# ALRhub/fancy_gym

Measured on AMD Instinct MI355X. Metric: MP trajectories/sec (7-DoF, 5 basis, 100 steps) at 1/2/4/8 GPUs; % roofline, higher is better.
Workload: dtype f32; 1 GPU; cfg2: ProDMP 7-DoF, 5 basis(+goal), 100 steps, exp phase tau=1.5, alpha=10; trajectory (pos, vel) + PD tracking-controller actions, fused; batch_per_gpu=4096, global_batch=4096, launch=hipgraph

## Files before the change

fancy_gym_amd/_lib.py:

```python
from __future__ import annotations

import ctypes as C
import os
from typing import Optional

_HERE = os.path.dirname(os.path.abspath(__file__))
LIB_PATH = os.environ.get("MPK_LIB") or os.path.join(_HERE, "libmpk.so")

MPK_ABI_VERSION = 4
MP_TYPES = {"promp": 0, "dmp": 1, "prodmp": 2}
PHASE_TYPES = {"linear": 0, "exp": 1}
BASIS_TYPES = {"rbf": 0, "zero_rbf": 1, "prodmp": 2}
CTRL_TYPES = {"motor": 0, "velocity": 1, "position": 2}
PLANT_TYPES = {"static": 0, "double_integrator": 1, "velocity_direct": 2}

MPK_EINVAL, MPK_ENOTIMPL, MPK_EHIP, MPK_ERANGE, MPK_ENODEV, MPK_ECOMM = -1, -2, -3, -4, -5, -6
MPK_COMM_ID_BYTES = 128
MPK_LOGPROB_MAX_OBS = 64
MPK_OPT_AUTO = -1
RELATIVE_GOAL_MODES = {"before_scale": 0, "after_scale": 1}
GOAL_OFFSET_MODES = {"ignore": 0, "add": 1}
SINGLE_RBF_MODES = {"unit_gap": 0, "refuse": 1}
DMP_FIRST_SAMPLE_MODES = {"init": 0, "step": 1}
REWARD_TYPES = {None: 0, "none": 0, "simple_reacher": 1}
AGG_MODES = {"sum": 0, "mean": 1, "last": 2}
OPTION_KEYS = ("mapping", "bulk", "quad", "pd_quad", "write_through", "ipw", "phase", "phase_table", "phase_chunk",
               "pd_simple", "split", "lds_pad", "pipe", "flat", "phase_flat", "ring", "ring_np", "ring_ns", "ring_m", "ring_dbg", "ring_parts", "tiles_wpb", "serial_order", "ring_nc", "pd_generic", "dmp_response", "ablations", "ring_tb", "pd_helper", "phase_waves", "phase_split", "phase_pipe", "pd_pipe", "hole_sampled", "vjp_generic")


class MPKLibraryError(RuntimeError):
    """libmpk.so is missing / failed to load / reported a HIP failure."""


class mpk_config(C.Structure):
    _fields_ = [
        ("abi_version", C.c_int32), ("device", C.c_int32),
        ("mp_type", C.c_int32), ("phase_type", C.c_int32), ("basis_type", C.c_int32),
        ("num_dof", C.c_int32), ("num_basis", C.c_int32), ("num_basis_outside", C.c_int32),
        ("num_basis_zero_start", C.c_int32), ("num_basis_zero_goal", C.c_int32),
        ("learn_tau", C.c_int32), ("learn_delay", C.c_int32),
        ("auto_scale_basis", C.c_int32), ("relative_goal", C.c_int32),
        ("disable_goal", C.c_int32), ("disable_weights", C.c_int32),
        ("pre_compute_length_factor", C.c_int32),
        ("relative_goal_mode", C.c_int32), ("goal_offset_mode", C.c_int32), ("single_rbf_mode", C.c_int32),
        ("dmp_first_sample", C.c_int32), ("reserved0", C.c_int32),
        ("tau", C.c_double), ("delay", C.c_double), ("alpha_phase", C.c_double),
        ("tau_bound", C.c_double * 2), ("delay_bound", C.c_double * 2),
        ("basis_bandwidth_factor", C.c_double), ("basis_alpha", C.c_double), ("basis_dt", C.c_double),
        ("weights_scale", C.c_double), ("goal_scale", C.c_double), ("dmp_alpha", C.c_double),
        ("dt", C.c_double), ("duration", C.c_double), ("goal_offset", C.c_double),
# ... 116 lines not shown
    "mpk_reacher_reset": (C.c_int, [_vp, C.POINTER(mpk_reacher_reset_task), _vp, _vp, _vp, _vp, _vp, _vp, _vp, _vp, _vp, _vp,
                                    _i32, _vp]),
    "mpk_reacher_observation": (C.c_int, [_vp, C.POINTER(mpk_obs_cfg), _vp, _vp, _vp, _vp, _vp, _i32, _vp]),
    "mpk_reacher_step_observations": (C.c_int, [_vp, C.POINTER(mpk_obs_cfg), C.POINTER(mpk_rollout_cfg), _vp, _vp, _vp, _vp, _vp, _vp,
                                                _vp, _vp, _vp, _vp, _i32, _i32, _vp]),
    "mpk_replan_advance": (C.c_int, [_vp, _vp, _vp, _vp, _vp, _i32, _i32, _i32, _i32, _i32, _vp]),
    "mpk_traj_validity": (C.c_int, [_vp, _vp, _vp, _vp, _vp, _i32, _vp, _vp, _vp, _i32, _i32, _vp]),
    "mpk_traj_validity_penalty": (C.c_int, [_vp, _vp, _vp, _vp, _vp, _i32, _vp, _vp, _vp, _vp, _i32, _i32, _vp]),
    "mpk_prodmp_tables": (C.c_int, [_vp, _vp, _vp, _vp, _vp, _vp, _vp, _vp]),
    "mpk_prodmp_indices": (C.c_int, [_vp, _dbl, _vp, _vp, _vp]),
    "mpk_scaled_basis": (C.c_int, [_vp, _vp, _i32, _vp, _vp]),
    "mpk_selftest_division": (C.c_int, [_vp, C.c_float, C.c_uint32, C.c_uint64, C.POINTER(C.c_uint64), _vp]),
    "mpk_host_prodmp_tables": (C.c_int, [C.POINTER(mpk_config), _vp, _vp, _vp, _vp, _vp, _vp, _vp, _vp]),
    "mpk_host_rbf": (C.c_int, [C.POINTER(mpk_config), _vp, _vp]),
    "mpk_host_times": (C.c_int, [_dbl, _dbl, _vp, _i32]),
    "mpk_host_num_params": (C.c_int, [C.POINTER(mpk_config)]),
    "mpk_comm_unique_id": (C.c_int, [_vp]),
    "mpk_comm_create": (C.c_int, [_vp, _i32, _i32, _i32, C.POINTER(_vp)]),
    "mpk_comm_rank": (C.c_int, [_vp]),
    "mpk_comm_world": (C.c_int, [_vp]),
    "mpk_allgather": (C.c_int, [_vp, _vp, _vp, C.c_int64, _vp]),
    "mpk_comm_destroy": (None, [_vp]),
    "mpk_last_kernel": (C.c_char_p, [_vp]),
    "mpk_reacher_autoreset": (C.c_int, [_vp, C.POINTER(mpk_reacher_reset_task), C.POINTER(mpk_obs_cfg), _vp, _vp, _vp, _vp, _vp, _vp,
                                        _vp, _vp, _vp, _vp, _vp, _vp, _vp, _vp, _i32, _vp]),
    "mpk_reacher_env_step": (C.c_int, [_vp, C.POINTER(mpk_env_step_task), C.POINTER(mpk_reacher_reset_task), _vp, _vp, _vp, _vp, _vp,
                                       _vp, _vp, _vp, _vp, _vp, _vp, _vp, _vp, _vp, _vp, _i32, _vp]),
    "mpk_trajectory_vjp": (C.c_int, [_vp, _vp, _vp, _dbl, _vp, _vp, _vp, _i32, _vp]),
    "mpk_reacher_rollout_vjp": (C.c_int, [_vp, C.POINTER(mpk_rollout_cfg), _vp, _vp, _vp, _vp, _vp, _vp, _vp, _i32, _vp, _vp, _vp,
                                          _vp, _vp, _vp, _vp, _vp, _i32, _i32, _vp]),
    "mpk_episode_return_vjp": (C.c_int, [_vp, _vp, _vp, _vp, _dbl, C.POINTER(mpk_rollout_cfg), _vp, _vp, _vp, _vp, _vp, _i32, _i32,
                                         _vp, _vp, _vp, _vp, _vp, _vp, _vp, _vp, _vp, _vp, _vp, _i32, _vp]),
    "mpk_hole_reacher_rollout_vjp": (C.c_int, [_vp, C.POINTER(mpk_rollout_cfg), _vp, _vp, _vp, _vp, _vp, _vp, C.POINTER(mpk_hole_task),
                                               _vp, _vp, _i32, _vp, _vp, _vp, _vp, _vp, _vp, _vp, _vp, _vp, _i32, _i32, _vp]),
    "mpk_reacher_rollout_vjp_cond": (C.c_int, [_vp, C.POINTER(mpk_rollout_cfg), _vp, _vp, _vp, _vp, _vp, _vp, _vp, _i32, _vp, _vp, _vp,
                                               _vp, _vp, _vp, _vp, _vp, _vp, _vp, _i32, _i32, _vp]),
    "mpk_episode_return_vjp_cond": (C.c_int, [_vp, _vp, _vp, _vp, _dbl, C.POINTER(mpk_rollout_cfg), _vp, _vp, _vp, _vp, _vp, _i32, _i32,
                                              _vp, _vp, _vp, _vp, _vp, _vp, _vp, _vp, _vp, _vp, _vp, _vp, _vp, _i32, _vp]),
    "mpk_hole_reacher_rollout_vjp_cond": (C.c_int, [_vp, C.POINTER(mpk_rollout_cfg), _vp, _vp, _vp, _vp, _vp, _vp,
                                                    C.POINTER(mpk_hole_task), _vp, _vp, _i32, _vp, _vp, _vp, _vp, _vp, _vp, _vp, _vp, _vp,
                                                    _vp, _vp, _i32, _i32, _vp]),
    "mpk_trajectory_fit": (C.c_int, [_vp, _vp, _vp, _vp, _vp, _dbl, _dbl, _vp, _i32, _vp]),
    "mpk_trajectory_phase_fit": (C.c_int, [_vp, _vp, _vp, _vp, _vp, _vp, _dbl, _dbl, _vp, _i32, _vp]),
    "mpk_fit_status": (C.c_int, [_vp, C.POINTER(C.c_int32), _vp]),
    "mpk_trajectory_std": (C.c_int, [_vp, _vp, _dbl, _vp, _vp, _i32, _vp]),
    "mpk_trajectory_condition": (C.c_int, [_vp, _vp, _vp, _vp, _vp, _dbl, C.POINTER(C.c_int32), _i32, _vp, _vp, _vp, _vp, _vp, _vp,
# ... 117 lines not shown
```

fancy_gym_amd/csrc/mpk_host.cpp:

```cpp
#include <hip/hip_runtime.h>
#include <dlfcn.h>

#include <cmath>
#include <cstdio>
#include <cstring>
#include <limits>
#include <map>
#include <mutex>
#include <set>

#include "mpk_internal.h"

namespace mpk {

static thread_local std::string g_err;
void set_error(const std::string& msg) { g_err = msg; }

const char* cond_variant_name(const char* plain) {
    static std::mutex m;
    static std::set<std::string> pool;
    std::lock_guard<std::mutex> lock(m);
    return pool.insert(std::string(plain) + " + cond").first->c_str();
}

// ... 181 lines not shown
    double* d_tab = nullptr;
    std::vector<float> rows32;
    float* d_rows32 = nullptr;
    int rows32_stride = 0;
    float* d_times = nullptr;
    int32_t* d_flag = nullptr;
    unsigned* d_tickets = nullptr;
    unsigned ticket_next = 0;
    std::vector<unsigned> ticket_free;
    std::map<std::pair<unsigned long long, uintptr_t>, unsigned> ticket_of;
    std::mutex ticket_mu;
    int* h_fault = nullptr;
    int* d_fault = nullptr;
    int32_t* d_idx = nullptr;
    int idx_cap = 0;
    static constexpr int kCache = 64;
    CacheEntry cache[kCache];
    DevCfg dev_resp{};
    bool resp_ok = false;
    CacheEntry cache_resp[kCache];
    std::string kernel_name_buf;
    uint64_t stamp = 0;
    const char* last_kernel = "";
    Tuning tune;
    float* d_pre = nullptr;
    size_t pre_cap = 0;
    static constexpr int kFitCache = 16;
    FitEntry fit_cache[kFitCache];
    int32_t* d_fit_status = nullptr;
};

static Tuning effective_tuning(const Handle* h);

static int check_cfg(const mpk_config& c) {
    if (c.abi_version != MPK_ABI_VERSION) { set_error("mpk_config.abi_version mismatch"); return MPK_EINVAL; }
    if (c.mp_type < 0 || c.mp_type > 2) { set_error("unknown mp_type"); return MPK_EINVAL; }
    if (c.phase_type < 0 || c.phase_type > 1) { set_error("unknown phase_type"); return MPK_EINVAL; }
    if (c.basis_type < 0 || c.basis_type > 2) { set_error("unknown basis_type"); return MPK_EINVAL; }
    if (c.num_dof < 0) { set_error("num_dof must be >= 0"); return MPK_EINVAL; }
    if (c.num_basis < 1) { set_error("num_basis must be >= 1 (basis length 0 is not implemented upstream)"); return MPK_EINVAL; }
    if (c.basis_type == MPK_BASIS_PRODMP && c.phase_type != MPK_PHASE_EXP) {
        set_error("prodmp basis requires the exp phase generator");
        return MPK_EINVAL;
    }
    if ((c.mp_type == MPK_MP_PRODMP) != (c.basis_type == MPK_BASIS_PRODMP)) {
        set_error("prodmp trajectory generator and prodmp basis generator must be used together");
// ... 434 lines not shown
    return prealloc_cache(h);
}

namespace {
struct OptKey { const char* name; int Tuning::*field; int64_t lo, hi; };
const OptKey kOptKeys[] = {
    {"mapping", &Tuning::mapping, 0, 2},         {"bulk", &Tuning::bulk, 0, 2},
    {"quad", &Tuning::quad, 0, 4},               {"pd_quad", &Tuning::pd_quad, 0, 3},
    {"write_through", &Tuning::write_through, 0, 1}, {"ipw", &Tuning::ipw, 0, 1 << 20},
    {"phase", &Tuning::phase, 0, 1},             {"phase_table", &Tuning::phase_table, 0, 1},
    {"phase_chunk", &Tuning::phase_chunk, 0, 16}, {"pd_simple", &Tuning::pd_simple, 0, 1},
    {"split", &Tuning::split, 0, 1},             {"lds_pad", &Tuning::lds_pad, 0, 48},
    {"pipe", &Tuning::pipe, 0, 1},               {"flat", &Tuning::flat, 0, 1},
    {"phase_flat", &Tuning::phase_flat, 0, 1},   {"ring", &Tuning::ring, 0, 2},
    {"ring_np", &Tuning::ring_np, 1, 14},        {"ring_ns", &Tuning::ring_ns, 1, 8},
    {"ring_m", &Tuning::ring_m, 1, 8},           {"ring_dbg", &Tuning::ring_dbg, 0, 255},
    {"ring_parts", &Tuning::ring_parts, 1, 8},   {"tiles_wpb", &Tuning::tiles_wpb, 1, 8},
    {"serial_order", &Tuning::serial_order, 0, 2}, {"ring_nc", &Tuning::ring_nc, 1, 6},
    {"pd_generic", &Tuning::pd_generic, 0, 1},   {"dmp_response", &Tuning::dmp_response, 0, 1},
    {"ablations", &Tuning::ablations, 0, 1},     {"ring_tb", &Tuning::ring_tb, 1, 64},
    {"pd_helper", &Tuning::pd_helper, 0, 1},     {"phase_waves", &Tuning::phase_waves, 1, 32},
    {"phase_split", &Tuning::phase_split, 1, 64},   {"phase_pipe", &Tuning::phase_pipe, 0, 1},
    {"pd_pipe", &Tuning::pd_pipe, 0, 1},         {"hole_sampled", &Tuning::hole_sampled, 0, 1},
    {"vjp_generic", &Tuning::vjp_generic, 0, 1},
};
const OptKey* find_opt(const char* key) {
    if (!key) return nullptr;
    for (const OptKey& k : kOptKeys)
        if (std::strcmp(k.name, key) == 0) return &k;
    return nullptr;
}
}

namespace mpk {
static Tuning effective_tuning(const Handle* h) {
    Tuning t = g_tune;
    for (const OptKey& k : kOptKeys)
        if (h->tune.*(k.field) >= 0) t.*(k.field) = h->tune.*(k.field);
    return t;
}
}

int mpk_set_option(mpk_handle hh, const char* key, int64_t value) {
    const OptKey* k = find_opt(key);
    if (!k) { set_error(std::string("unknown option key: ") + (key ? key : "(null)")); return MPK_EINVAL; }
    if (value != MPK_OPT_AUTO && (value < k->lo || value > k->hi)) {
        set_error(std::string("option value out of range for ") + key);
// ... 114 lines not shown
    out->check_td = g->check_tau_delay ? 1 : 0;
    if (out->check_td && h->dev.P < 2) { set_error("validity gate: check_tau_delay needs at least two parameters per episode"); return MPK_EINVAL; }
    out->tau_b[0] = g->tau_bound[0]; out->tau_b[1] = g->tau_bound[1];
    out->delay_b[0] = g->delay_bound[0]; out->delay_b[1] = g->delay_bound[1];
    out->raw_params = g->raw_params; out->valid = g->valid; out->penalty = g->penalty;
    return MPK_OK;
}

static int fill_replan(const mpk_replan_state* st, const float* init_pos, const float* init_vel, ReplanDev* rp) {
    if (!st || !st->traj_steps || !st->plan_steps || !st->done || !st->seg_len) { set_error("NULL replanning state"); return MPK_EINVAL; }
    if ((st->cond_pos == nullptr) != (st->cond_vel == nullptr)) { set_error("cond_pos and cond_vel go together"); return MPK_EINVAL; }
    if (st->every < 1 || st->horizon < 1) { set_error("every and horizon must be >= 1"); return MPK_EINVAL; }
    if (st->cond_pos && (st->cond_pos == init_pos || st->cond_vel == init_vel)) { set_error("cond_pos / cond_vel must not alias init_pos / init_vel"); return MPK_EINVAL; }
    rp->traj_steps = st->traj_steps; rp->plan_steps = st->plan_steps; rp->done = st->done; rp->seg_len = st->seg_len;
    rp->done_out = st->done_out; rp->cond_pos = st->cond_pos; rp->cond_vel = st->cond_vel;
    rp->every = st->every; rp->max_planning_times = st->max_planning_times; rp->horizon = st->horizon;
    return MPK_OK;
}

static LaunchSite launch_site(Handle* h, const Tuning& tune, void* stream) {
    LaunchSite at;
    at.num_cu = h->num_cu; at.tune = tune; at.stream = stream; at.kernel_name = &h->last_kernel;
    at.fault = h->d_fault; at.range_flag = h->d_flag;
    return at;
}

static void report_kernel(Handle* h, const char* name, bool resp) {
    h->kernel_name_buf = name;
    const size_t at = resp ? h->kernel_name_buf.find("prodmp") : std::string::npos;
    if (at != std::string::npos) h->kernel_name_buf.replace(at, 6, "dmp_resp");
    h->last_kernel = h->kernel_name_buf.c_str();
}

static int phase_fused_common(Handle* h, const TrajRequest& q, void* stream) {
    if (!q.params || !q.init_pos || !q.init_vel) { set_error("NULL buffer"); return MPK_EINVAL; }
    if (const int fr = pending_ring_fault(h); fr != MPK_OK) return fr;
    return launch_phase_fused(h->dev, q, launch_site(h, effective_tuning(h), stream));
}

static int traj_common(Handle* h, const TrajRequest& req, void* stream) {
    if (req.B < 0) { set_error("B must be >= 0"); return MPK_EINVAL; }
    if (req.B == 0 || h->dev.D == 0) return MPK_OK;
    if (!req.params || !req.init_pos || !req.init_vel || !req.pos || !req.vel) { set_error("NULL buffer"); return MPK_EINVAL; }
    MPK_ON_DEVICE(h->cfg.device);
    if (const int fr = pending_ring_fault(h); fr != MPK_OK) return fr;
    TrajRequest q = req;
// ... 1399 lines not shown
    if (count < 0) { set_error("count must be >= 0"); return MPK_EINVAL; }
    if (count == 0) return MPK_OK;
    if (!send || !recv) { set_error("NULL buffer"); return MPK_EINVAL; }
    Comm* c = reinterpret_cast<Comm*>(cc);
    MPK_ON_DEVICE(c->device);
    const int rc = rccl().AllGather(send, recv, (size_t)count, kNcclFloat, c->nccl, (hipStream_t)stream);
    if (rc != 0) return rccl_fail("ncclAllGather", rc);
    return MPK_OK;
}

void mpk_comm_destroy(mpk_comm cc) {
    if (!cc) return;
    Comm* c = reinterpret_cast<Comm*>(cc);
    DeviceGuard guard(c->device);
    if (c->nccl) (void)rccl().CommDestroy(c->nccl);
    delete c;
}

const char* mpk_last_kernel(mpk_handle hh) {
    if (!hh) return "";
    return reinterpret_cast<Handle*>(hh)->last_kernel;
}

}
```

fancy_gym_amd/csrc/mpk_internal.h:

```cpp
#pragma once
#include <cstdint>
#include <string>
#include <vector>

#include "mpk.h"

namespace mpk {

constexpr int kMaxKP = 16;
constexpr int kMaxD = 16;
constexpr int kMaxDofArgs = 32;

struct HostTables {
    int n_total = 0;
    std::vector<double> centers, bw;
    int n_pc = 0;
    float scaled_dt = 0.f;
    std::vector<double> y1, y2, dy1, dy2, pos_basis, vel_basis, scale;
};

void build_rbf(const mpk_config& c, HostTables& t);
void build_prodmp(const mpk_config& c, HostTables& t);
std::vector<float> build_times(double duration, int T);
int steps_for(double duration, double dt);

struct Tuning {
    int mapping = -1, bulk = -1, quad = -1, pd_quad = -1, write_through = -1, ipw = -1, phase = -1, phase_table = -1,
        phase_chunk = -1, pd_simple = -1, split = -1, lds_pad = -1, pipe = -1, flat = -1, phase_flat = -1,
        ring = -1, ring_np = -1, ring_ns = -1, ring_m = -1, ring_dbg = -1, ring_parts = -1, tiles_wpb = -1, serial_order = -1, ring_nc = -1,
        pd_generic = -1, dmp_response = -1, ablations = -1, ring_tb = -1, pd_helper = -1, phase_waves = -1, phase_split = -1, phase_pipe = -1, pd_pipe = -1,
        hole_sampled = -1, vjp_generic = -1;
};

struct DevCfg {
    int mp_type, phase_type, basis_type;
    int D, nb, n_total, zs;
    int KT, KP;
    int P, Kloc, off;
    int T;
    int learn_tau, learn_delay, relative_goal, disable_goal, disable_weights;
    int rbf_uniform;
    int relgoal_before_scale;
    int dmp_resp;
    int goal_off_on;
    float goal_offset;
    int n_pc, len_factor;
    float tau, delay, alpha_phase, scaled_dt;
    float tau_lo, tau_hi, delay_lo, delay_hi;
    float ws, gs, dmp_alpha, dmp_beta;
    const double* tab;
    const float* rows32;
    int rows32_stride;
    const float* base_times;
    float t_last;
// ... 50 lines not shown
    const int32_t* step0 = nullptr;
    double* ret = nullptr;
    int32_t* seg_out = nullptr;
};
struct TrajRequest {
    const float *params = nullptr, *init_pos = nullptr, *init_vel = nullptr;
    const float* init_time = nullptr;
    float init_time_shared = 0.f;
    float *pos = nullptr, *vel = nullptr, *actions = nullptr;
    const RolloutDev* rc = nullptr;
    const double *c_pos = nullptr, *c_vel = nullptr;
    double *q_state = nullptr, *qd_state = nullptr;
    const int32_t* n_steps = nullptr;
    const ReplanDev* rp = nullptr;
    const GateDev* gate = nullptr;
    EpisodeAsk ep;
    int B = 0;
};
struct LaunchSite {
    int num_cu = 0;
    Tuning tune;
    void* stream = nullptr;
    const char** kernel_name = nullptr;
    unsigned* ticket = nullptr;
    int* fault = nullptr;
    int32_t* range_flag = nullptr;
};

int launch_build_shared(const DevCfg& c, float init_time, const SharedTables& st, int32_t* idx_out,
                        int32_t* range_flag, void* stream);
int launch_traj_shared(const DevCfg& c, const SharedTables& st, const TrajRequest& q, const LaunchSite& at);
int launch_episode_return(const DevCfg& c, const SharedTables& st, const TrajRequest& q, const LaunchSite& at);
int launch_reward_aggregate(const double* rewards, const int32_t* seg_len, int agg, double* out, int B, int T, void* stream);
int launch_traj_wide(const DevCfg& c, const SharedTables& st, const TrajRequest& q, const LaunchSite& at);
int launch_traj_vjp(const DevCfg& c, const SharedTables& st, const float* g_pos, const float* g_vel, float* g_params, float* g_init_pos,
                    float* g_init_vel, int B, int num_cu, void* stream, const char** kernel_name, const Tuning& tune);
int launch_traj_rows(const DevCfg& c, const TrajRequest& q, const LaunchSite& at);
int launch_pd_rollout(const RolloutDev& rc, int D, const float* des_pos, const float* des_vel, double* q,
                      double* qd, const int32_t* n_steps, float* actions, int B, int T, void* stream,
                      const Tuning& tune, int* fault = nullptr);
bool phase_fused_capable(const DevCfg& c);
int launch_phase_fused(const DevCfg& c, const TrajRequest& q, const LaunchSite& at);
int fast_rows_floats(const DevCfg& c);
int fast_rows_stride(const DevCfg& c);
int launch_fast_rows_table(const DevCfg& c, float* out, void* stream);
int launch_dmp_prestep(const DevCfg& c, const TrajRequest& q, float* pos1, float* vel1, void* stream);
// ... 215 lines not shown
```

fancy_gym_amd/csrc/mpk_tile.h:

```cpp
#pragma once
#include "mpk_dev.h"

namespace mpk {

struct TrajArgs {
    DevCfg c;
    const float* A;
    const float* aux;
    int TS;
    const float* params;
    const float* init_pos;
    const float* init_vel;
    float* pos;
    float* vel;
    float* actions;
    const double* c_pos;
    const double* c_vel;
    int B, sh, G, vec_ok;
    int pitch, cps, shifted, td3;
    unsigned inv_cps;
    unsigned nrt_magic;
    int gstride;
    int wt;
    int flat_img;
// ... 625 lines not shown
                const f32x2 v2 = {head ? d1[2] : d1[0], head ? d1[3] : d1[1]};
                if (SP) store8<WT>(a.pos + go + o, p2);
                if (SV) store8<WT>(a.vel + go + o, v2);
                if (SA) {
                    const f32x2 a2 = {head ? d2[2] : d2[0], head ? d2[3] : d2[1]};
                    store8<WT>(a.actions + go + o, a2);
                }
            } else {
#pragma unroll
                for (int e = 0; e < 4; ++e) {
                    if (c0 + e >= lo && c0 + e < hi) {
                        if (SP) store4<WT>(a.pos + go + e, d0[e]);
                        if (SV) store4<WT>(a.vel + go + e, d1[e]);
                        if (SA) store4<WT>(a.actions + go + e, d2[e]);
                    }
                }
            }
        }
    } else {
        store_tile_generic(a.pos, a.vel, a.actions, MASK, a.B, T, D, L.NTW, sSt, lane, b0, rt, rows);
    }
}

template <int NST, int KM, bool WT>
__device__ __forceinline__ void tile_store(const TrajArgs& a, const LaneMap<KM>& L, const float* sSt, int lane,
                                           int b0, int rt, int rows) {
    tile_store_sel<(NST > 2 ? 7 : 3), KM, WT>(a, L, sSt, lane, b0, rt, rows);
}

__device__ __forceinline__ void demand_args(const TrajArgs& a, unsigned grid_x) {
    asm volatile("" ::"s"(grid_x), "s"(a.c.D), "s"(a.c.nb), "s"(a.c.KT), "s"(a.c.P), "s"(a.c.Kloc), "s"(a.c.off), "s"(a.c.T),
                 "s"(a.c.disable_weights), "s"(a.c.disable_goal), "s"(a.c.goal_off_on), "s"(a.A), "s"(a.aux), "s"(a.TS), "s"(a.params),
                 "s"(a.init_pos), "s"(a.init_vel), "s"(a.pos), "s"(a.vel), "s"(a.actions), "s"(a.c_pos), "s"(a.c_vel),
                 "s"(a.sh), "s"(a.G), "s"(a.vec_ok), "s"(a.pitch), "s"(a.cps), "s"(a.shifted), "s"(a.td3),
                 "s"(a.inv_cps), "s"(a.nrt_magic), "s"(a.gstride));
}

__device__ __forceinline__ void load_ds16(const float* __restrict__ p, float (&v)[16]) {
#pragma unroll
    for (int j = 0; j < 4; ++j) {
        const float4 x = reinterpret_cast<const float4*>(p)[j];
        v[4 * j] = x.x; v[4 * j + 1] = x.y; v[4 * j + 2] = x.z; v[4 * j + 3] = x.w;
    }
}

}
// ... 1 lines not shown
```

fancy_gym_amd/csrc/mpk_traj_family.hip:

```cpp
#include "mpk_traj_tiles.h"
#include "mpk_traj_stream.h"
#include "mpk_traj_flat.h"
#include "mpk_traj_quad.h"
#include "mpk_traj_pipe.h"
#include "mpk_traj_route.h"

namespace mpk {

#ifndef MPK_DEVICE_ONLY
template <int MP, int CT>
static int launch_traj_t(const TrajArgs& ta, const ActArgs& aa, const TrajRoute& r, void* stream) {
    auto go = [&](auto kern, unsigned threads, bool full_lds = false) {
        if (full_lds && r.lds > 48 * 1024) (void)allow_full_lds(kern);
        hipLaunchKernelGGL(kern, dim3(r.blocks), dim3(threads), r.lds, (hipStream_t)stream, ta, aa);
    };
    with_km(ta.c.KP / 4, [&](auto km) {
        constexpr int KM = decltype(km)::value;
        switch (r.family) {
            case TrajFamily::Pipe:
                if constexpr (MP != MPK_MP_DMP && CT >= 3) {
                    if (r.gate) go(k_traj_pipe<MP, CT, KM, false, true>, 320);
                    else if (r.lean) go(k_traj_pipe<MP, CT, KM, true>, 320);
                    else go(k_traj_pipe<MP, CT, KM, false>, 320);
                }
                break;
            case TrajFamily::Flat:
                if constexpr (MP != MPK_MP_DMP && CT < 3) go(k_traj_flat<MP, CT, KM>, 256, true);
                break;
            case TrajFamily::Split:
                if constexpr (MP != MPK_MP_DMP && CT >= 3)
                    with_flag(r.write_through, [&](auto wt) { go(k_traj_split<MP, CT, KM, decltype(wt)::value>, 256); });
                break;
            case TrajFamily::Quarter:
                if constexpr (MP == MPK_MP_DMP || CT >= 3) {
                    if (r.nq == 1) go(k_traj_quad<MP, CT, KM, 1>, 256);
                    else if (r.nq == 2) go(k_traj_quad<MP, CT, KM, 2>, 256);
                    else go(k_traj_quad<MP, CT, KM, 4>, 256);
                }
                break;
            case TrajFamily::Stream:
                with_flag(r.bulk, [&](auto bulk) { go(k_traj_stream<MP, CT, KM, decltype(bulk)::value>, 256, decltype(bulk)::value); });
                break;
            case TrajFamily::Tiles:
                if constexpr (MP != MPK_MP_DMP && CT < 3)
                    with_flag(r.write_through, [&](auto wt) { go(k_traj_tiles<MP, CT, KM, decltype(wt)::value>, (unsigned)ta.wpb * 64u); });
                break;
            default: break;
        }
    });
    MPK_LAUNCH_CHECK();
    return MPK_OK;
}

template <int MP>
int launch_traj_ct(const TrajArgs& ta, const ActArgs& aa, const TrajRoute& r, void* stream) {
    auto go = [&](auto ct) { return launch_traj_t<MP, decltype(ct)::value>(ta, aa, r, stream); };
    if constexpr (MP == MPK_MP_DMP) return go(std::integral_constant<int, -1>());
    else return r.family == TrajFamily::Pipe || r.family == TrajFamily::Split ? with_closed_ct(r.ct, go) : with_ct(r.ct, go);
}

#ifdef MPK_MP_UNIT
template int launch_traj_ct<MPK_MP_UNIT>(const TrajArgs&, const ActArgs&, const TrajRoute&, void*);
#else
template int launch_traj_ct<MPK_MP_PROMP>(const TrajArgs&, const ActArgs&, const TrajRoute&, void*);
template int launch_traj_ct<MPK_MP_DMP>(const TrajArgs&, const ActArgs&, const TrajRoute&, void*);
template int launch_traj_ct<MPK_MP_PRODMP>(const TrajArgs&, const ActArgs&, const TrajRoute&, void*);
#endif
#endif
// ... 3 lines not shown
```

fancy_gym_amd/csrc/mpk_traj_launch.hip:

```cpp
#include <cstdio>

#include "mpk_tile.h"
#include "mpk_traj_quad.h"
#include "mpk_traj_pipe.h"
#include "mpk_traj_stream.h"
#include "mpk_traj_ring.h"
#include "mpk_traj_route.h"

namespace mpk {

bool shared_tables_lean(const DevCfg& c) { return c.KP > kMaxKP || c.D > kMaxD; }

size_t shared_tables_floats(const DevCfg& c, int* TS, int* n_out) {
    const int TP = (c.T + 15) / 16 * 16;
    const int ts = ((TP + 15) / 32) * 32 + 16;
    const bool lean = shared_tables_lean(c);
    const int no = c.mp_type == MPK_MP_PRODMP ? 2 : (c.mp_type == MPK_MP_PROMP && !lean ? 3 : 1);
    *TS = ts;
    *n_out = no;
    return (lean ? 1 : 2) * (size_t)no * c.KP * ts;
}

__global__ void __launch_bounds__(256) k_build_shared(const DevCfg c, const float init_time, float* __restrict__ A,
                                                      float* __restrict__ aux, const int TS, const int n_out, const int lean,
// ... 524 lines not shown
    f.lds_flat = table_bytes + (size_t)4 * f.nst * f.flat_img * sizeof(float);
    f.flat_ok = !closed && !dmp && ptr_ok && TD % 4 == 0 && f.lds_flat <= kLdsHalf;
    f.flat_takes_it = !act && f.flat_ok && tune.flat != 0;
    f.stream_from = f.flat_takes_it && tune.bulk < 0 ? kFlatTrajBytes : kCachedBytes;
    f.serial = (dmp || closed) && !f.split;
    const bool open_episode_major = !dmp && !closed && (ov == 2 || tune.flat == 1 || tune.ring >= 1 || (ov != 1 && out_bytes > f.stream_from));
    const bool stream_fits = table_bytes + 4 * kStageFloats * sizeof(float) <= kLdsDefault;
    if (f.serial && !stream_fits) { set_error("trajectory too long for the episode-major kernel's LDS budget"); return MPK_ENOTIMPL; }
    f.episode_major = f.serial || (open_episode_major && stream_fits);

    r = TrajRoute{};
    r.ct = dmp ? -1 : ct;
    if (!(plan_ring_open(f, ta, r) || plan_ring_closed(f, ta, r) || plan_pipe(f, ta, r) || plan_quarter(f, ta, r))) {
        if (gated) return MPK_ENOTIMPL;
        if (!(plan_burst(f, ta, r) || plan_flat(f, ta, r) || plan_stream(f, ta, r))) plan_tiles(f, ta, r);
    }
    if (r.blocks < 1) r.blocks = 1;
    const bool tile_major = r.family == TrajFamily::Tiles || r.family == TrajFamily::Split;
    if (tile_major && ta.gstride <= 0) { set_error("internal: tile-major launch without its group stride"); return MPK_EINVAL; }
    bool wt = tune.write_through >= 0 ? tune.write_through != 0 : (tile_major || out_bytes <= kWtBytes);
    if ((double)B * c.T * c.D * 4.0 >= 2147483648.0) wt = false;
    r.write_through = tile_major && wt;
    ta.wt = !tile_major && wt ? 1 : 0;
    r.name = traj_kernel_name(r, gated && dmp ? MPK_MP_PROMP : c.mp_type, act, closed);
    return gated && dmp ? MPK_ENOTIMPL : MPK_OK;
}

int launch_traj_shared(const DevCfg& c, const SharedTables& st, const TrajRequest& q, const LaunchSite& at) {
    TrajArgs ta{};
    ActArgs aa{};
    TrajRoute r{};
    const int rc_ = plan_traj_shared(c, st, q, at.num_cu, at.tune, at.ticket, at.fault, ta, aa, r);
    if (r.name) *at.kernel_name = r.name;
    if (rc_ != MPK_OK) return rc_;
    switch (r.family) {
        case TrajFamily::RingOpen: case TrajFamily::RingClosed: case TrajFamily::Burst: case TrajFamily::FlatD:
            return by_mp_type(c.mp_type, [&](auto mp) { return launch_traj_ring<decltype(mp)::value>(ta, aa, r, at.stream); });
        default:
            return by_mp_type(c.mp_type, [&](auto mp) { return launch_traj_ct<decltype(mp)::value>(ta, aa, r, at.stream); });
    }
}
#endif

}
```

fancy_gym_amd/csrc/mpk_traj_route.h:

```cpp
#pragma once
#include "mpk_tile.h"

namespace mpk {

enum class TrajFamily : int {
    Tiles,
    Split,
    Stream,
    Flat,
    FlatD,
    Burst,
    Quarter,
    Pipe,
    RingOpen,
    RingClosed,
};

struct TrajRoute {
    TrajFamily family;
    int ct;
    bool write_through;
    bool bulk;
    int nq;
    bool lean, gate;
    int blocks;
    size_t lds;
    const char* name;
};

struct EpRoute {
    int ct, nq, rwd, blocks;
    size_t lds;
    const char* name;
};

#ifndef MPK_DEVICE_ONLY
int plan_traj_shared(const DevCfg& c, const SharedTables& st, const TrajRequest& q, int num_cu, const Tuning& tune, unsigned* ticket,
                     int* fault, TrajArgs& ta, ActArgs& aa, TrajRoute& r);
int plan_episode_return(const DevCfg& c, const SharedTables& st, const TrajRequest& q, int num_cu, const Tuning& tune, TrajArgs& ta,
                        ActArgs& aa, EpArgs& ea, EpRoute& r);

template <int MP>
int launch_traj_ct(const TrajArgs& ta, const ActArgs& aa, const TrajRoute& r, void* stream);
template <int MP>
// ... 61 lines not shown
```

fancy_gym_amd/csrc/mpk_traj_tiles.h:

```cpp
#pragma once
#include "mpk_tile.h"

namespace mpk {

template <int MP, int CT, int KM, bool WT>
__device__ __forceinline__ void tiles_body(const TrajArgs& a, float* smem, const unsigned bid, const unsigned nblk) {
    static_assert(MP != MPK_MP_DMP, "dmp runs in k_traj_stream");
    static_assert(CT < 3, "closed-loop rollouts run in k_traj_stream / k_traj_split");
    constexpr bool ACT = CT >= 0;
    constexpr int NOUT = MP == MPK_MP_PRODMP ? 2 : 3;
    constexpr int NST = 2 + (ACT ? 1 : 0);
    const DevCfg& c = a.c;
    const int lane = threadIdx.x & 63;
    const int wave = __builtin_amdgcn_readfirstlane(threadIdx.x >> 6);
    const int KP = 4 * KM, TS = a.TS, D = c.D, T = c.T;
    float* sSt = smem + wave * kStageFloats;
    const LaneMap<KM> L = make_lane_map<MP, KM>(a, lane);
    const int NRT = (T + 15) >> 4;
    const int nb8 = (int)(nblk >> 3);
    const int vb = (nblk & 7) == 0 ? (int)(bid & 7) * nb8 + (int)(bid >> 3) : (int)bid;
    const int wid = vb * a.wpb + wave;
    const int gstride = a.gstride;
    int g = a.nrt_magic ? (int)__umulhi((unsigned)wid, a.nrt_magic) : wid;
    const int rt = wid - g * NRT;
    if (g >= a.G) return;
    MPK_STAMP(1);
    GroupIn<KM> cur = load_group<MP, ACT, KM>(a, L, g);
    Gains kg{0.0, 0.0, 0.0, 0.0};
    if (ACT) kg = kernarg_gains(L.dvalid ? L.d : 0);
    float af[NOUT][KM];
#pragma unroll
    for (int j = 0; j < NOUT; ++j)
#pragma unroll
        for (int m = 0; m < KM; ++m) af[j][m] = a.A[(size_t)(j * KP + 4 * m + L.q) * TS + rt * 16 + L.col];
    float dtd[4] = {1.f, 1.f, 1.f, 1.f};
    if (MP == MPK_MP_PROMP) {
#pragma unroll
        for (int r = 0; r < 4; ++r) dtd[r] = a.aux[rt * 16 + 4 * L.q + r];
    }
    const int rows = min(16, T - rt * 16);

    float xb[KM];
    finish_group<KM>(L, cur, xb);
    double cp = cur.cp, cv = cur.cv;
    MPK_STAMP(2);
    while (g < a.G) {
        const int gn = g + gstride;
        const GroupIn<KM> nxt = load_group<MP, ACT, KM>(a, L, gn < a.G ? gn : g);
        f32x4 acc0 = {0.f, 0.f, 0.f, 0.f}, acc1 = {0.f, 0.f, 0.f, 0.f}, acc2 = {0.f, 0.f, 0.f, 0.f};
#pragma unroll
        for (int m = 0; m < KM; ++m) {
            acc0 = __builtin_amdgcn_mfma_f32_16x16x4f32(af[0][m], xb[m], acc0, 0, 0, 0);
            acc1 = __builtin_amdgcn_mfma_f32_16x16x4f32(af[1][m], xb[m], acc1, 0, 0, 0);
            if (NOUT > 2) acc2 = __builtin_amdgcn_mfma_f32_16x16x4f32(af[NOUT > 2 ? 2 : 0][m], xb[m], acc2, 0, 0, 0);
        }
        if (L.dvalid)
            tile_epilogue<MP, CT>(acc0, acc1, acc2, dtd, cp, cv, kg, sSt, L.wofs + ep_shift(a, g * L.NTW + L.bl), D);
        __builtin_amdgcn_wave_barrier();
        MPK_STAMP(10);
#if MPK_TILES_COLLECT_FIRST
        finish_group<KM>(L, nxt, xb);
        asm volatile("" : "+v"(xb[0]));
        tile_store<NST, KM, WT>(a, L, sSt, lane, g * L.NTW, rt, rows);
        __builtin_amdgcn_wave_barrier();
        MPK_STAMP(11);
#else
        tile_store<NST, KM, WT>(a, L, sSt, lane, g * L.NTW, rt, rows);
        __builtin_amdgcn_wave_barrier();
        MPK_STAMP(11);
        finish_group<KM>(L, nxt, xb);
#endif
        cp = nxt.cp; cv = nxt.cv;
        g = gn;
    }
#ifdef MPK_TRACE
    MPK_STAMP(20);
    asm volatile("s_waitcnt vmcnt(0)" ::: "memory");
    MPK_STAMP(21);
#endif
}

#ifndef MPK_TILES_OCC
#ifndef MPK_TILES_COLLECT_FIRST
#define MPK_TILES_COLLECT_FIRST 0
#endif
#define MPK_TILES_OCC 7
#endif
template <int MP, int CT, int KM, bool WT>
__global__ void __launch_bounds__(256, (KM <= 2 ? MPK_TILES_OCC : 1)) k_traj_tiles(const TrajArgs a, const ActArgs act) {
    __shared__ __attribute__((aligned(16))) float smem[4 * kStageFloats];
    demand_args(a, gridDim.x);
    tiles_body<MP, CT, KM, WT>(a, smem, blockIdx.x, gridDim.x);
}

template <int MP, int CT, int KM, bool WT>
__device__ __forceinline__ void serial_body(const TrajArgs& a, const float* __restrict__ At,
                                            const float* __restrict__ aux, float* smem) {
    static_assert(CT >= 3, "closed loop only");
    constexpr int KP = 4 * KM;
    constexpr int NOUT = MP == MPK_MP_PRODMP ? 2 : 3;
    constexpr int RS = NOUT * KP;
    const DevCfg& c = a.c;
    const int lane = threadIdx.x & 63;
    const int wave = __builtin_amdgcn_readfirstlane(threadIdx.x >> 6);
    const int D = c.D, T = c.T, B = a.B, P = c.P;
    const int DP = 1 << a.sh, EPW = 64 >> a.sh;
    const int e = lane >> a.sh, d = lane & (DP - 1);
    const bool dvalid = d < D;
    float* sAct = smem + wave * (kStageFloats + 16 * RS);
    const int NRT = (T + 15) >> 4;
    const int units = (B + EPW - 1) / EPW;
    const int ustride = (int)a.ser_blocks * 4;
    const Gains gn = kernarg_gains(dvalid ? d : 0);
    const double pgd = gn.pg, dgd = gn.dg, lod = __builtin_canonicalize(gn.lo), hid = __builtin_canonicalize(gn.hi),
                 dtp = a.plant_dt;
// ... 178 lines not shown
```

fancy_gym_amd/engine.py:

```python
from __future__ import annotations

import ctypes as C
import os
from typing import Optional, Sequence, Tuple, Union

import numpy as np
import torch

from . import _lib
from ._lib import (BASIS_TYPES, CTRL_TYPES, MP_TYPES, PHASE_TYPES, PLANT_TYPES, MPKLibraryError, mpk_config,
                   mpk_rollout_cfg)

_INF = float("inf")


def _dptr(t: Optional[torch.Tensor]) -> Optional[int]:
    return None if t is None else t.data_ptr()


def _dvec(x, n: int):
    a = np.ascontiguousarray(np.broadcast_to(np.asarray(x, dtype=np.float64), (n,)))
    return a.ctypes.data_as(C.POINTER(C.c_double)), a


# ... 1749 lines not shown
        K = self.config.num_basis + 1
        arrs = [np.empty(n, np.float64) for _ in range(4)] + [np.empty((n, K), np.float64) for _ in range(2)] + \
               [np.empty(K, np.float64)]
        _lib.check(self._lib.mpk_prodmp_tables(self._h, *[a.ctypes.data for a in arrs]))
        return dict(zip(("y1", "y2", "dy1", "dy2", "pos_basis", "vel_basis", "scale"), arrs))

    def prodmp_indices(self, init_time: float = 0.0):
        T = self.num_steps
        idx = np.empty(T, np.int32)
        ib = np.empty(1, np.int32)
        _lib.check(self._lib.mpk_prodmp_indices(self._h, float(init_time), idx.ctypes.data, ib.ctypes.data,
                                                self._stream()))
        return idx, int(ib[0])

    def scaled_basis(self, times) -> np.ndarray:
        t = np.ascontiguousarray(np.asarray(times, np.float32).reshape(-1))
        K = self.config.num_basis + (1 if self.mp_type == "prodmp" else 0)
        out = np.empty((t.shape[0], K), np.float32)
        _lib.check(self._lib.mpk_scaled_basis(self._h, t.ctypes.data, int(t.shape[0]), out.ctypes.data, self._stream()))
        return out

    def last_kernel(self) -> str:
        return self._lib.mpk_last_kernel(self._h).decode()
```

include/mpk.h:

```cpp
#ifndef MPK_H
#define MPK_H

#include <stdint.h>

#ifdef __cplusplus
extern "C" {
#endif

#define MPK_ABI_VERSION 4

#define MPK_OK            0
#define MPK_EINVAL       -1
#define MPK_ENOTIMPL     -2
#define MPK_EHIP         -3
#define MPK_ERANGE       -4
#define MPK_ENODEV       -5
#define MPK_ECOMM        -6

#define MPK_MP_PROMP   0
#define MPK_MP_DMP     1
#define MPK_MP_PRODMP  2
#define MPK_PHASE_LINEAR 0
#define MPK_PHASE_EXP    1
#define MPK_BASIS_RBF       0
// ... 258 lines not shown
int mpk_prodmp_indices(mpk_handle h, double init_time, int32_t* idx, int32_t* idx_init, void* stream);

int mpk_scaled_basis(mpk_handle h, const float* times, int32_t n, float* basis, void* stream);

int mpk_selftest_division(mpk_handle h, float divisor, uint32_t first_bits, uint64_t count, uint64_t* mismatches,
                          void* stream);

int mpk_host_prodmp_tables(const mpk_config* cfg, double* y1, double* y2, double* dy1, double* dy2,
                           double* pos_basis, double* vel_basis, double* scale, float* scaled_dt);
int mpk_host_rbf(const mpk_config* cfg, double* centers, double* bw);
int mpk_host_times(double duration, double dt, float* times, int32_t cap);
int mpk_host_num_params(const mpk_config* cfg);

#define MPK_COMM_ID_BYTES 128
typedef struct mpk_comm_s* mpk_comm;
int mpk_comm_unique_id(uint8_t* id);
int mpk_comm_create(const uint8_t* id, int32_t rank, int32_t world, int32_t device, mpk_comm* out);
int mpk_comm_rank(mpk_comm c);
int mpk_comm_world(mpk_comm c);
int mpk_allgather(mpk_comm c, const float* send, float* recv, int64_t count, void* stream);
void mpk_comm_destroy(mpk_comm c);

const char* mpk_last_kernel(mpk_handle h);

int mpk_reacher_autoreset(mpk_handle h, const mpk_reacher_reset_task* task, const mpk_obs_cfg* cfg, const uint64_t* seeds,
                          mpk_nprng_state* rng, double* q, double* qd, float* cond_pos, float* cond_vel, int32_t* traj_steps,
                          int32_t* plan_steps, uint8_t* done, double* task_io, const uint8_t* mask, uint8_t* reset_mask,
                          float* final_obs, float* obs, int32_t B, void* stream);

typedef struct mpk_env_step_task {
    int32_t env;
    int32_t n_links;
    double  dt;
    int32_t max_episode_steps;
    int32_t autoreset;
    mpk_hole_task hole;
    int64_t reserved[2];
} mpk_env_step_task;
int mpk_reacher_env_step(mpk_handle h, const mpk_env_step_task* step, const mpk_reacher_reset_task* reset, const float* actions,
                         mpk_nprng_state* rng, double* q, double* qd, int32_t* traj_steps, double* task_io, double* reward_state,
                         double* reward, uint8_t* terminated, uint8_t* truncated, uint8_t* is_collided, uint8_t* is_success,
                         uint8_t* reset_mask, float* final_obs, float* obs, int32_t B, void* stream);

int mpk_trajectory_vjp(mpk_handle h, const float* g_pos, const float* g_vel, double init_time_shared,
                       float* g_params, float* g_init_pos, float* g_init_vel, int32_t B, void* stream);

// ... 82 lines not shown
```

Measured before the change: 486.4 million trajectories/s.

## Add aligned-window tile store path for write-through trajectory tiles

Adds an aligned variant of the tiles kernel. Each row tile overlaps its neighbours so that global stores of pos, vel and actions fall on 16-float aligned boundaries and can be written as full 16-byte vectors without partial-line writes. The staging pitch, the epilogue write offset and the A-matrix row base are remapped to match. The path is gated by a tuning key that defaults to auto, and by shape and pointer-alignment checks. The overlapping windows recompute some rows and add conditions to the launch plan.

New measurement: 507.0 million trajectories/s (median of 5 runs). +4.2%, better.

```diff
diff --git a/fancy_gym_amd/_lib.py b/fancy_gym_amd/_lib.py
--- a/fancy_gym_amd/_lib.py
+++ b/fancy_gym_amd/_lib.py
@@ -25,7 +25,7 @@
 REWARD_TYPES = {None: 0, "none": 0, "simple_reacher": 1}
 AGG_MODES = {"sum": 0, "mean": 1, "last": 2}
 OPTION_KEYS = ("mapping", "bulk", "quad", "pd_quad", "write_through", "ipw", "phase", "phase_table", "phase_chunk",
-               "pd_simple", "split", "lds_pad", "pipe", "flat", "phase_flat", "ring", "ring_np", "ring_ns", "ring_m", "ring_dbg", "ring_parts", "tiles_wpb", "serial_order", "ring_nc", "pd_generic", "dmp_response", "ablations", "ring_tb", "pd_helper", "phase_waves", "phase_split", "phase_pipe", "pd_pipe", "hole_sampled", "vjp_generic")
+               "pd_simple", "split", "lds_pad", "pipe", "flat", "phase_flat", "ring", "ring_np", "ring_ns", "ring_m", "ring_dbg", "ring_parts", "tiles_wpb", "serial_order", "ring_nc", "pd_generic", "dmp_response", "ablations", "ring_tb", "pd_helper", "phase_waves", "phase_split", "phase_pipe", "pd_pipe", "hole_sampled", "vjp_generic", "tiles_align")
 
 
 class MPKLibraryError(RuntimeError):
@@ -188,6 +188,7 @@
     "mpk_allgather": (C.c_int, [_vp, _vp, _vp, C.c_int64, _vp]),
     "mpk_comm_destroy": (None, [_vp]),
     "mpk_last_kernel": (C.c_char_p, [_vp]),
+    "mpk_last_tiles_aligned": (C.c_int, [_vp]),
     "mpk_reacher_autoreset": (C.c_int, [_vp, C.POINTER(mpk_reacher_reset_task), C.POINTER(mpk_obs_cfg), _vp, _vp, _vp, _vp, _vp, _vp,
                                         _vp, _vp, _vp, _vp, _vp, _vp, _vp, _vp, _i32, _vp]),
     "mpk_reacher_env_step": (C.c_int, [_vp, C.POINTER(mpk_env_step_task), C.POINTER(mpk_reacher_reset_task), _vp, _vp, _vp, _vp, _vp,
diff --git a/fancy_gym_amd/csrc/mpk_host.cpp b/fancy_gym_amd/csrc/mpk_host.cpp
--- a/fancy_gym_amd/csrc/mpk_host.cpp
+++ b/fancy_gym_amd/csrc/mpk_host.cpp
@@ -227,6 +227,7 @@
     std::string kernel_name_buf;
     uint64_t stamp = 0;
     const char* last_kernel = "";
+    int last_tiles_aligned = 0;
     Tuning tune;
     float* d_pre = nullptr;
     size_t pre_cap = 0;
@@ -707,7 +708,7 @@
     {"pd_helper", &Tuning::pd_helper, 0, 1},     {"phase_waves", &Tuning::phase_waves, 1, 32},
     {"phase_split", &Tuning::phase_split, 1, 64},   {"phase_pipe", &Tuning::phase_pipe, 0, 1},
     {"pd_pipe", &Tuning::pd_pipe, 0, 1},         {"hole_sampled", &Tuning::hole_sampled, 0, 1},
-    {"vjp_generic", &Tuning::vjp_generic, 0, 1},
+    {"vjp_generic", &Tuning::vjp_generic, 0, 1}, {"tiles_align", &Tuning::tiles_align, 0, 1},
 };
 const OptKey* find_opt(const char* key) {
     if (!key) return nullptr;
@@ -868,6 +869,7 @@
     LaunchSite at;
     at.num_cu = h->num_cu; at.tune = tune; at.stream = stream; at.kernel_name = &h->last_kernel;
     at.fault = h->d_fault; at.range_flag = h->d_flag;
+    h->last_tiles_aligned = 0; at.tiles_aligned = &h->last_tiles_aligned;
     return at;
 }
 
@@ -2313,4 +2315,8 @@
     return reinterpret_cast<Handle*>(hh)->last_kernel;
 }
 
-}
+int32_t mpk_last_tiles_aligned(mpk_handle hh) {
+    return hh ? reinterpret_cast<Handle*>(hh)->last_tiles_aligned : 0;
+}
+
+}
diff --git a/fancy_gym_amd/csrc/mpk_internal.h b/fancy_gym_amd/csrc/mpk_internal.h
--- a/fancy_gym_amd/csrc/mpk_internal.h
+++ b/fancy_gym_amd/csrc/mpk_internal.h
@@ -29,7 +29,7 @@
         phase_chunk = -1, pd_simple = -1, split = -1, lds_pad = -1, pipe = -1, flat = -1, phase_flat = -1,
         ring = -1, ring_np = -1, ring_ns = -1, ring_m = -1, ring_dbg = -1, ring_parts = -1, tiles_wpb = -1, serial_order = -1, ring_nc = -1,
         pd_generic = -1, dmp_response = -1, ablations = -1, ring_tb = -1, pd_helper = -1, phase_waves = -1, phase_split = -1, phase_pipe = -1, pd_pipe = -1,
-        hole_sampled = -1, vjp_generic = -1;
+        hole_sampled = -1, vjp_generic = -1, tiles_align = -1;
 };
 
 struct DevCfg {
@@ -126,6 +126,7 @@
     Tuning tune;
     void* stream = nullptr;
     const char** kernel_name = nullptr;
+    int* tiles_aligned = nullptr;
     unsigned* ticket = nullptr;
     int* fault = nullptr;
     int32_t* range_flag = nullptr;
diff --git a/fancy_gym_amd/csrc/mpk_tile.h b/fancy_gym_amd/csrc/mpk_tile.h
--- a/fancy_gym_amd/csrc/mpk_tile.h
+++ b/fancy_gym_amd/csrc/mpk_tile.h
@@ -671,6 +671,31 @@
     }
 }
 
+__host__ __device__ __forceinline__ int aligned_tile_rows(int D) { return 16 - (12 + D - 1) / D; }
+template <int MASK, int KM, bool WT>
+__device__ __forceinline__ void tile_store_aligned(const TrajArgs& a, const LaneMap<KM>& L, const float* sSt, int b0, int r0,
+                                                   bool last) {
+    constexpr bool SA = (MASK & 4) != 0;
+    const int D = a.c.D, TD = a.c.T * D;
+    const int bb = b0 + L.sseg;
+    const int phi = (int)(((unsigned)bb * (unsigned)TD) & 15u);
+    const int t0 = r0 * D, t1 = t0 + aligned_tile_rows(D) * D;
+    const int lo = r0 == 0 ? 0 : ((t0 + phi + 15) & ~15) - phi;
+    const int hi = last ? TD : ((t1 + phi + 15) & ~15) - phi;
+    const int f = lo + L.w4;
+    if (L.sseg < L.NTW && bb < a.B && f + 4 <= hi) {
+        const unsigned ro = L.rofs + (unsigned)((t0 & 3) + lo - t0);
+        const size_t go = (size_t)bb * TD + f;
+        const f32x4 d0 = *reinterpret_cast<const f32x4*>(sSt + ro);
+        const f32x4 d1 = *reinterpret_cast<const f32x4*>(sSt + kStageStride + ro);
+        f32x4 d2 = {0.f, 0.f, 0.f, 0.f};
+        if (SA) d2 = *reinterpret_cast<const f32x4*>(sSt + 2 * kStageStride + ro);
+        store16<WT>(a.pos + go, d0);
+        store16<WT>(a.vel + go, d1);
+        if (SA) store16<WT>(a.actions + go, d2);
+    }
+}
+
 template <int NST, int KM, bool WT>
 __device__ __forceinline__ void tile_store(const TrajArgs& a, const LaneMap<KM>& L, const float* sSt, int lane,
                                            int b0, int rt, int rows) {
diff --git a/fancy_gym_amd/csrc/mpk_traj_family.hip b/fancy_gym_amd/csrc/mpk_traj_family.hip
--- a/fancy_gym_amd/csrc/mpk_traj_family.hip
+++ b/fancy_gym_amd/csrc/mpk_traj_family.hip
@@ -42,8 +42,12 @@
                 with_flag(r.bulk, [&](auto bulk) { go(k_traj_stream<MP, CT, KM, decltype(bulk)::value>, 256, decltype(bulk)::value); });
                 break;
             case TrajFamily::Tiles:
-                if constexpr (MP != MPK_MP_DMP && CT < 3)
+                if constexpr (MP != MPK_MP_DMP && CT < 3) {
+                    if constexpr (KM <= 2) {
+                        if (r.tiles_align) { go(k_traj_tiles<MP, CT, KM, true, true>, (unsigned)ta.wpb * 64u); break; }
+                    }
                     with_flag(r.write_through, [&](auto wt) { go(k_traj_tiles<MP, CT, KM, decltype(wt)::value>, (unsigned)ta.wpb * 64u); });
+                }
                 break;
             default: break;
         }
diff --git a/fancy_gym_amd/csrc/mpk_traj_launch.hip b/fancy_gym_amd/csrc/mpk_traj_launch.hip
--- a/fancy_gym_amd/csrc/mpk_traj_launch.hip
+++ b/fancy_gym_amd/csrc/mpk_traj_launch.hip
@@ -570,6 +570,14 @@
     if ((double)B * c.T * c.D * 4.0 >= 2147483648.0) wt = false;
     r.write_through = tile_major && wt;
     ta.wt = !tile_major && wt ? 1 : 0;
+    {
+        auto aligned64 = [](const void* p) { return (reinterpret_cast<uintptr_t>(p) & 63u) == 0; };
+        const bool shape = ta.vec_ok && !ta.shifted && c.KP <= 8 && c.D >= 3 && c.D <= 7 && NTW * (SEG + 4) <= kStageStride &&
+                           (f.NRT - 1) * aligned_tile_rows(c.D) + 16 >= c.T &&
+                           aligned64(q.pos) && aligned64(q.vel) && (!act || aligned64(q.actions));
+        r.tiles_align = r.family == TrajFamily::Tiles && r.write_through && shape && tune.tiles_align != 0;
+        if (r.tiles_align) ta.pitch = SEG + 4;
+    }
     r.name = traj_kernel_name(r, gated && dmp ? MPK_MP_PROMP : c.mp_type, act, closed);
     return gated && dmp ? MPK_ENOTIMPL : MPK_OK;
 }
@@ -580,6 +588,7 @@
     TrajRoute r{};
     const int rc_ = plan_traj_shared(c, st, q, at.num_cu, at.tune, at.ticket, at.fault, ta, aa, r);
     if (r.name) *at.kernel_name = r.name;
+    if (at.tiles_aligned) *at.tiles_aligned = rc_ == MPK_OK && r.tiles_align ? 1 : 0;
     if (rc_ != MPK_OK) return rc_;
     switch (r.family) {
         case TrajFamily::RingOpen: case TrajFamily::RingClosed: case TrajFamily::Burst: case TrajFamily::FlatD:
diff --git a/fancy_gym_amd/csrc/mpk_traj_route.h b/fancy_gym_amd/csrc/mpk_traj_route.h
--- a/fancy_gym_amd/csrc/mpk_traj_route.h
+++ b/fancy_gym_amd/csrc/mpk_traj_route.h
@@ -20,6 +20,7 @@
     TrajFamily family;
     int ct;
     bool write_through;
+    bool tiles_align;
     bool bulk;
     int nq;
     bool lean, gate;
diff --git a/fancy_gym_amd/csrc/mpk_traj_tiles.h b/fancy_gym_amd/csrc/mpk_traj_tiles.h
--- a/fancy_gym_amd/csrc/mpk_traj_tiles.h
+++ b/fancy_gym_amd/csrc/mpk_traj_tiles.h
@@ -3,7 +3,7 @@
 
 namespace mpk {
 
-template <int MP, int CT, int KM, bool WT>
+template <int MP, int CT, int KM, bool WT, bool AL = false>
 __device__ __forceinline__ void tiles_body(const TrajArgs& a, float* smem, const unsigned bid, const unsigned nblk) {
     static_assert(MP != MPK_MP_DMP, "dmp runs in k_traj_stream");
     static_assert(CT < 3, "closed-loop rollouts run in k_traj_stream / k_traj_split");
@@ -28,17 +28,19 @@
     GroupIn<KM> cur = load_group<MP, ACT, KM>(a, L, g);
     Gains kg{0.0, 0.0, 0.0, 0.0};
     if (ACT) kg = kernarg_gains(L.dvalid ? L.d : 0);
+    const int r0 = AL ? rt * aligned_tile_rows(D) : rt * 16;
     float af[NOUT][KM];
 #pragma unroll
     for (int j = 0; j < NOUT; ++j)
 #pragma unroll
-        for (int m = 0; m < KM; ++m) af[j][m] = a.A[(size_t)(j * KP + 4 * m + L.q) * TS + rt * 16 + L.col];
+        for (int m = 0; m < KM; ++m) af[j][m] = a.A[(size_t)(j * KP + 4 * m + L.q) * TS + r0 + L.col];
     float dtd[4] = {1.f, 1.f, 1.f, 1.f};
     if (MP == MPK_MP_PROMP) {
 #pragma unroll
-        for (int r = 0; r < 4; ++r) dtd[r] = a.aux[rt * 16 + 4 * L.q + r];
+        for (int r = 0; r < 4; ++r) dtd[r] = a.aux[r0 + 4 * L.q + r];
     }
     const int rows = min(16, T - rt * 16);
+    const unsigned wmain = AL ? L.wofs + ((unsigned)(r0 * D) & 3u) : L.wofs;
 
     float xb[KM];
     finish_group<KM>(L, cur, xb);
@@ -55,17 +57,19 @@
             if (NOUT > 2) acc2 = __builtin_amdgcn_mfma_f32_16x16x4f32(af[NOUT > 2 ? 2 : 0][m], xb[m], acc2, 0, 0, 0);
         }
         if (L.dvalid)
-            tile_epilogue<MP, CT>(acc0, acc1, acc2, dtd, cp, cv, kg, sSt, L.wofs + ep_shift(a, g * L.NTW + L.bl), D);
+            tile_epilogue<MP, CT>(acc0, acc1, acc2, dtd, cp, cv, kg, sSt, AL ? wmain : L.wofs + ep_shift(a, g * L.NTW + L.bl), D);
         __builtin_amdgcn_wave_barrier();
         MPK_STAMP(10);
 #if MPK_TILES_COLLECT_FIRST
         finish_group<KM>(L, nxt, xb);
         asm volatile("" : "+v"(xb[0]));
-        tile_store<NST, KM, WT>(a, L, sSt, lane, g * L.NTW, rt, rows);
+        if (AL) tile_store_aligned<(NST > 2 ? 7 : 3), KM, WT>(a, L, sSt, g * L.NTW, r0, rt == NRT - 1);
+        else tile_store<NST, KM, WT>(a, L, sSt, lane, g * L.NTW, rt, rows);
         __builtin_amdgcn_wave_barrier();
         MPK_STAMP(11);
 #else
-        tile_store<NST, KM, WT>(a, L, sSt, lane, g * L.NTW, rt, rows);
+        if (AL) tile_store_aligned<(NST > 2 ? 7 : 3), KM, WT>(a, L, sSt, g * L.NTW, r0, rt == NRT - 1);
+        else tile_store<NST, KM, WT>(a, L, sSt, lane, g * L.NTW, rt, rows);
         __builtin_amdgcn_wave_barrier();
         MPK_STAMP(11);
         finish_group<KM>(L, nxt, xb);
@@ -86,11 +90,12 @@
 #endif
 #define MPK_TILES_OCC 7
 #endif
-template <int MP, int CT, int KM, bool WT>
+template <int MP, int CT, int KM, bool WT, bool AL = false>
 __global__ void __launch_bounds__(256, (KM <= 2 ? MPK_TILES_OCC : 1)) k_traj_tiles(const TrajArgs a, const ActArgs act) {
+    static_assert(!AL || (WT && KM <= 2), "aligned windows: write-through launches of up to 8 columns");
     __shared__ __attribute__((aligned(16))) float smem[4 * kStageFloats];
     demand_args(a, gridDim.x);
-    tiles_body<MP, CT, KM, WT>(a, smem, blockIdx.x, gridDim.x);
+    tiles_body<MP, CT, KM, WT, AL>(a, smem, blockIdx.x, gridDim.x);
 }
 
 template <int MP, int CT, int KM, bool WT>
diff --git a/fancy_gym_amd/engine.py b/fancy_gym_amd/engine.py
--- a/fancy_gym_amd/engine.py
+++ b/fancy_gym_amd/engine.py
@@ -1795,3 +1795,6 @@
 
     def last_kernel(self) -> str:
         return self._lib.mpk_last_kernel(self._h).decode()
+
+    def last_tiles_aligned(self) -> bool:
+        return bool(self._lib.mpk_last_tiles_aligned(self._h))
diff --git a/include/mpk.h b/include/mpk.h
--- a/include/mpk.h
+++ b/include/mpk.h
@@ -304,6 +304,7 @@
 void mpk_comm_destroy(mpk_comm c);
 
 const char* mpk_last_kernel(mpk_handle h);
+int32_t mpk_last_tiles_aligned(mpk_handle h);
 
 int mpk_reacher_autoreset(mpk_handle h, const mpk_reacher_reset_task* task, const mpk_obs_cfg* cfg, const uint64_t* seeds,
                           mpk_nprng_state* rng, double* q, double* qd, float* cond_pos, float* cond_vel, int32_t* traj_steps,
```
